# WangWen-Believer/DR-SLAM

Measured on AMD Instinct MI355X. Metric: RGB-D frames/sec (extract+match) at 640x480, higher is better.
Workload: dtype u8; 1 GPU; 640x480 synthetic RGB-D (TUM3 intrinsics), ORB extract 1000/1.2/8/20/7 + SearchByProjection(frame k, frame k-1, th=15) on consecutive frames; BASELINE config 2; batch_per_gpu=512, batches_in_flight_per_gpu=3, distinct_resident_input_batches_per_gpu=3, sequence_frames_per_rank=64

## Files before the change

dr_slam_amd/csrc/orb_kernels.hip:

```cpp
#include "drfe_internal.h"
#include "../../include/drfe_math.h"

#define WAVE 64

__device__ __forceinline__ int reflect101(int p, int n)
{
    if (p < 0) p = -p;
    if (p >= n) p = 2 * (n - 1) - p;
    return p;
}


#define PYR0_ROWS 2
__global__ __launch_bounds__(256) void k_pyr_level0_wide(const DevLevel L, int pyrSlotBytes, const uint8_t* __restrict__ gray,
                                                         size_t frameStride, size_t rowStride, int x16First, int x16Last,
                                                         uint8_t* __restrict__ pyr)
{
    const int slot = blockIdx.z;
    const int y0 = (blockIdx.y * 4 + threadIdx.y) * PYR0_ROWS;
    const int x16 = x16First + (blockIdx.x * 64 + threadIdx.x) * 16;
    const int bh = L.h + 2 * DRFE_EDGE;
    if (y0 >= bh || x16 > x16Last) return;
    const int sx = x16 - DRFE_EDGE;
    const uint8_t* frame = gray + (size_t)slot * frameStride;
    uint4 out[PYR0_ROWS];
#pragma unroll
    for (int r = 0; r < PYR0_ROWS; r++) {
        const int y = min(y0 + r, bh - 1);
        const uint8_t* src = frame + (size_t)reflect101(y - DRFE_EDGE, L.h) * rowStride;
        const uint4 A = *reinterpret_cast<const uint4*>(src + (sx - 13));
        const uint4 B = *reinterpret_cast<const uint4*>(src + (sx + 3));
        out[r] = make_uint4(__builtin_amdgcn_alignbyte(B.x, A.w, 1), __builtin_amdgcn_alignbyte(B.y, B.x, 1),
                            __builtin_amdgcn_alignbyte(B.z, B.y, 1), __builtin_amdgcn_alignbyte(B.w, B.z, 1));
    }
    uint8_t* dst = pyr + (size_t)slot * pyrSlotBytes + L.pyrOff + x16;
#pragma unroll
    for (int r = 0; r < PYR0_ROWS; r++)
        if (y0 + r < bh) *reinterpret_cast<uint4*>(dst + (size_t)(y0 + r) * L.pyrPitch) = out[r];
}

__global__ __launch_bounds__(256) void k_pyr_level0_edge(const DevLevel L, int pyrSlotBytes, const uint8_t* __restrict__ gray,
                                                         size_t frameStride, size_t rowStride, int leftEnd, int rightBegin,
                                                         uint8_t* __restrict__ pyr)
{
    const int slot = blockIdx.y;
    const int nLeft = leftEnd / 4, nPer = nLeft + (L.pyrPitch - rightBegin) / 4;
    const int bw = L.w + 2 * DRFE_EDGE, bh = L.h + 2 * DRFE_EDGE;
    const int item = blockIdx.x * 256 + threadIdx.x;
    if (item >= nPer * bh) return;
    const int y = item / nPer, t = item - y * nPer;
    const int x4 = t < nLeft ? t * 4 : rightBegin + (t - nLeft) * 4;
    const uint8_t* src = gray + (size_t)slot * frameStride + (size_t)reflect101(y - DRFE_EDGE, L.h) * rowStride;
    uint32_t o = 0;
#pragma unroll
    for (int k = 0; k < 4; k++) {
        const int x = x4 + k;
        uint32_t v = 0;
        if (x < bw) v = src[reflect101(x - DRFE_EDGE, L.w)];
        o |= v << (8 * k);
    }
    *reinterpret_cast<uint32_t*>(pyr + (size_t)slot * pyrSlotBytes + L.pyrOff + (size_t)y * L.pyrPitch + x4) = o;
}

__device__ __forceinline__ uint32_t pick_byte(uint32_t d0, uint32_t d1, uint32_t d2, int o)
{
    const uint32_t w = o < 4 ? d0 : (o < 8 ? d1 : d2);
    return (w >> (8 * (o & 3))) & 0xFFu;
}

#define PYR_ROWS 4
__global__ __launch_bounds__(256) void k_pyr_resize(const DevLevel L, const DevLevel P, int pyrSlotBytes,
                                                    const ResizeTap* __restrict__ taps, uint8_t* __restrict__ pyr)
{
    const int slot = blockIdx.z;
    const int y0 = (blockIdx.y * 4 + threadIdx.y) * PYR_ROWS;
    const int x4 = (blockIdx.x * 64 + threadIdx.x) * 4;
    const int bh = L.h + 2 * DRFE_EDGE;
    if (y0 >= bh || x4 >= L.pyrPitch) return;
    uint8_t* base = pyr + (size_t)slot * pyrSlotBytes;
    const uint4 tya = *reinterpret_cast<const uint4*>(taps + L.ytabOff + y0);
    const uint4 tyb = *reinterpret_cast<const uint4*>(taps + L.ytabOff + y0 + 2);
    const uint4 ta = *reinterpret_cast<const uint4*>(taps + L.xtabOff + x4);
    const uint4 tb = *reinterpret_cast<const uint4*>(taps + L.xtabOff + x4 + 2);
    const uint32_t syp[PYR_ROWS] = {tya.x, tya.z, tyb.x, tyb.z}, wyp[PYR_ROWS] = {tya.y, tya.w, tyb.y, tyb.w};
    const uint32_t sp[4] = {ta.x, ta.z, tb.x, tb.z};
    const uint32_t wp[4] = {ta.y, ta.w, tb.y, tb.w};
    int lo = 0xFFFF;
#pragma unroll
    for (int k = 0; k < 4; k++) lo = min(lo, (int)(sp[k] & 0xFFFF));
    const int ws = (lo + DRFE_EDGE) & ~3;
    const uint8_t* srcw = base + P.pyrOff + (size_t)DRFE_EDGE * P.pyrPitch + ws;
    uint32_t a[PYR_ROWS][3], c[PYR_ROWS][3];
#pragma unroll
    for (int r = 0; r < PYR_ROWS; r++) {
        const uint32_t* R0 = reinterpret_cast<const uint32_t*>(srcw + (size_t)(syp[r] & 0xFFFF) * P.pyrPitch);
        const uint32_t* R1 = reinterpret_cast<const uint32_t*>(srcw + (size_t)(syp[r] >> 16) * P.pyrPitch);
        a[r][0] = R0[0]; a[r][1] = R0[1]; a[r][2] = R0[2];
        c[r][0] = R1[0]; c[r][1] = R1[1]; c[r][2] = R1[2];
    }
    int o0[4], o1[4], w0[4], w1[4];
#pragma unroll
    for (int k = 0; k < 4; k++) {
        o0[k] = (int)(sp[k] & 0xFFFF) + DRFE_EDGE - ws; o1[k] = (int)(sp[k] >> 16) + DRFE_EDGE - ws;
        w0[k] = (int)(short)(wp[k] & 0xFFFF); w1[k] = (int)(short)(wp[k] >> 16);
    }
#pragma unroll
    for (int r = 0; r < PYR_ROWS; r++) {
        if (y0 + r >= bh) break;
        const int b0 = (int)(short)(wyp[r] & 0xFFFF), b1 = (int)(short)(wyp[r] >> 16);
        uint32_t out = 0;
#pragma unroll
        for (int k = 0; k < 4; k++) {
            const int h0 = (int)pick_byte(a[r][0], a[r][1], a[r][2], o0[k]) * w0[k] + (int)pick_byte(a[r][0], a[r][1], a[r][2], o1[k]) * w1[k];
            const int h1 = (int)pick_byte(c[r][0], c[r][1], c[r][2], o0[k]) * w0[k] + (int)pick_byte(c[r][0], c[r][1], c[r][2], o1[k]) * w1[k];
            int v = (((b0 * (h0 >> 4)) >> 16) + ((b1 * (h1 >> 4)) >> 16) + 2) >> 2;
            v = min(255, max(0, v));
            out |= (uint32_t)v << (8 * k);
        }
        *reinterpret_cast<uint32_t*>(base + L.pyrOff + (size_t)(y0 + r) * L.pyrPitch + x4) = out;
    }
}

template <int FILL>
__global__ __launch_bounds__(256) void k_pyr_resize_tile(const DevLevel L, const DevLevel P, int pyrSlotBytes,
                                                         const ResizeTap* __restrict__ taps, uint8_t* __restrict__ pyr,
                                                         uint32_t magicBlocks)
{
    extern __shared__ __attribute__((aligned(16))) uint8_t tile[];
    int bx, slot;
    drfe_xcd_swizzle_2d(magicBlocks, bx, slot);
    bx = __builtin_amdgcn_readfirstlane(bx); slot = __builtin_amdgcn_readfirstlane(slot);
    const int tid = threadIdx.x;
    uint8_t* const base = pyr + (size_t)slot * pyrSlotBytes;
    const uint32_t winp = ((const __attribute__((address_space(4))) uint32_t*)taps)[2 * (L.rzWinOff + bx)];
    const struct { uint32_t s0, s1; } win = {winp & 0xFFFFu, winp >> 16};
    const uint32_t nItems = (uint32_t)(L.rzGroups * L.rzCols);
    uint32_t item = (uint32_t)(bx * DRFE_RESIZE_BLOCK + tid);
    const bool active = item < nItems;
    if (!active) item = nItems - 1;
    auto divm = [](uint32_t n, uint32_t d, uint32_t magic) { const uint32_t q = __umulhi(n, magic); return q * d > n ? q - 1 : q; };
    const uint32_t g = divm(item, (uint32_t)L.rzCols, L.rzColsMagic);
    const int y0 = L.rzRow0 + 4 * (int)g, x4 = 4 * (int)(item - g * (uint32_t)L.rzCols);
    const uint8_t* const tb8 = reinterpret_cast<const uint8_t*>(taps);
    const uint32_t tyo = (uint32_t)(L.ytabOff + y0) * 8u, txo = (uint32_t)(L.xtabOff + x4) * 8u;
    const uint2 t0 = *reinterpret_cast<const uint2*>(tb8 + tyo), t1 = *reinterpret_cast<const uint2*>(tb8 + (tyo + 8u));
    const uint2 t2 = *reinterpret_cast<const uint2*>(tb8 + (tyo + 16u)), t3 = *reinterpret_cast<const uint2*>(tb8 + (tyo + 24u));
    const uint4 ta = *reinterpret_cast<const uint4*>(tb8 + txo);
    const uint4 tb = *reinterpret_cast<const uint4*>(tb8 + (txo + 16u));
    {
        const uint8_t* const srcw = base + P.pyrOff + (uint32_t)((int)win.s0 * P.pyrPitch + (int)win.s1);
        const uint32_t nq = (uint32_t)(L.rzRows * L.rzWq), tpitch = (uint32_t)L.rzWq * 16u;
        uint4 v[FILL];
        uint32_t dst[FILL];
#pragma unroll
        for (int k = 0; k < FILL; k++) {
            const uint32_t j = (uint32_t)tid + (uint32_t)(k * DRFE_RESIZE_BLOCK), jc = j < nq ? j : 0u;
            const uint32_t r = divm(jc, (uint32_t)L.rzWq, L.rzWqMagic), q = jc - r * (uint32_t)L.rzWq;
            v[k] = *reinterpret_cast<const uint4*>(srcw + (__umul24(r, (uint32_t)P.pyrPitch) + q * 16u));
            dst[k] = j < nq ? __umul24(r, tpitch) + q * 16u : nq * 16u;
        }
#pragma unroll
        for (int k = 0; k < FILL; k++) *reinterpret_cast<uint4*>(&tile[dst[k]]) = v[k];
    }
    __syncthreads();
    if (!active) return;
    const uint32_t tpitch = (uint32_t)L.rzWq * 16u;
    const uint32_t sp[4] = {ta.x, ta.z, tb.x, tb.z}, wp[4] = {ta.y, ta.w, tb.y, tb.w};
    int o[4];
#pragma unroll
    for (int k = 0; k < 4; k++) o[k] = (int)(sp[k] & 0xFFFFu) + DRFE_EDGE - (int)win.s1;
    const uint32_t p01 = (uint32_t)min(o[0], o[1]) & ~3u, p23 = (uint32_t)min(o[2], o[3]) & ~3u;
    uint32_t sel[4];
#pragma unroll
    for (int k = 0; k < 4; k++) {
        const uint32_t rel = (uint32_t)o[k] - (k < 2 ? p01 : p23);
        sel[k] = rel | ((rel + 1u) << 16) | 0x0C000C00u;
    }
    typedef unsigned short u16x2v __attribute__((ext_vector_type(2)));
    auto hrow = [&](int srow, uint32_t (&H)[4]) {
        const uint32_t* A = reinterpret_cast<const uint32_t*>(&tile[(uint32_t)srow * tpitch + p01]);
        const uint32_t* C = reinterpret_cast<const uint32_t*>(&tile[(uint32_t)srow * tpitch + p23]);
        const uint32_t a0 = A[0], a1 = A[1], c0 = C[0], c1 = C[1];
        const uint32_t pr[4] = {__builtin_amdgcn_perm(a1, a0, sel[0]), __builtin_amdgcn_perm(a1, a0, sel[1]),
                                __builtin_amdgcn_perm(c1, c0, sel[2]), __builtin_amdgcn_perm(c1, c0, sel[3])};
#pragma unroll
        for (int k = 0; k < 4; k++)
            H[k] = __builtin_amdgcn_udot2(__builtin_bit_cast(u16x2v, pr[k]), __builtin_bit_cast(u16x2v, wp[k]), 0u, false) >> 4;
    };
    uint8_t* const dstLevel = base + L.pyrOff;
    const uint2 typ[4] = {t0, t1, t2, t3};
    const int rowEnd = L.rzRow0 + 4 * L.rzGroups;
    int prevB = -1;
    uint32_t Hp[4] = {0, 0, 0, 0};
#pragma unroll
    for (int r = 0; r < 4; r++) {
        const uint32_t sy = typ[r].x, wy2 = typ[r].y;
        const int a = (int)(sy & 0xFFFFu) + DRFE_EDGE - (int)win.s0, b = (int)(sy >> 16) + DRFE_EDGE - (int)win.s0;
        uint32_t Ha[4], Hb[4];
        if (a == prevB) {
#pragma unroll
            for (int k = 0; k < 4; k++) Ha[k] = Hp[k];
        } else hrow(a, Ha);
        if (b == a) {
#pragma unroll
            for (int k = 0; k < 4; k++) Hb[k] = Ha[k];
        } else hrow(b, Hb);
        const uint32_t b0s = wy2 << 16, b1s = wy2 & 0xFFFF0000u;
        uint32_t sm[4];
#pragma unroll
        for (int k = 0; k < 4; k++) sm[k] = __umulhi(Ha[k], b0s) + __umulhi(Hb[k], b1s) + 2u;
        const u16x2v two = {2, 2};
        const uint32_t q01 = __builtin_bit_cast(uint32_t, __builtin_bit_cast(u16x2v, sm[0] | (sm[1] << 16)) >> two);
        const uint32_t q23 = __builtin_bit_cast(uint32_t, __builtin_bit_cast(u16x2v, sm[2] | (sm[3] << 16)) >> two);
        const uint32_t out = __builtin_amdgcn_perm(q23, q01, 0x06040200u);
        const int y = y0 + r, p = y - DRFE_EDGE;
        *reinterpret_cast<uint32_t*>(dstLevel + (uint32_t)(__umul24((uint32_t)y, (uint32_t)L.pyrPitch) + (uint32_t)x4)) = out;
        if (p >= 1 && p <= DRFE_EDGE && DRFE_EDGE - p < L.rzRow0)
            *reinterpret_cast<uint32_t*>(dstLevel + (uint32_t)(__umul24((uint32_t)(DRFE_EDGE - p), (uint32_t)L.pyrPitch) + (uint32_t)x4)) = out;
        const int yb = DRFE_EDGE + 2 * (L.h - 1) - p;
        if (p >= L.h - 1 - DRFE_EDGE && p <= L.h - 2 && yb >= rowEnd)
            *reinterpret_cast<uint32_t*>(dstLevel + (uint32_t)(__umul24((uint32_t)yb, (uint32_t)L.pyrPitch) + (uint32_t)x4)) = out;
        prevB = b;
#pragma unroll
        for (int k = 0; k < 4; k++) Hp[k] = Hb[k];
    }
}


typedef short s16x2 __attribute__((ext_vector_type(2)));
__device__ __forceinline__ s16x2 pk2(uint32_t lo, uint32_t hi) { return __builtin_bit_cast(s16x2, lo | (hi << 16)); }
__device__ __forceinline__ s16x2 pmin(s16x2 a, s16x2 b) { return __builtin_elementwise_min(a, b); }
__device__ __forceinline__ s16x2 pmax(s16x2 a, s16x2 b) { return __builtin_elementwise_max(a, b); }
typedef unsigned short u16x2 __attribute__((ext_vector_type(2)));
__device__ __forceinline__ u16x2 umax2(u16x2 a, u16x2 b) { return __builtin_elementwise_max(a, b); }
__device__ __forceinline__ u16x2 umin2(u16x2 a, u16x2 b) { return __builtin_elementwise_min(a, b); }

typedef _Float16 h16x2 __attribute__((ext_vector_type(2)));
__device__ __forceinline__ h16x2 hpk(uint32_t lo, uint32_t hi) { return __builtin_bit_cast(h16x2, lo | (hi << 16)); }
__device__ __forceinline__ h16x2 hmin(h16x2 a, h16x2 b) { return __builtin_elementwise_minimum(a, b); }
__device__ __forceinline__ h16x2 hmax(h16x2 a, h16x2 b) { return __builtin_elementwise_maximum(a, b); }
__device__ __forceinline__ h16x2 hmin3(h16x2 a, h16x2 b, h16x2 c) { return hmin(hmin(a, b), c); }
__device__ __forceinline__ h16x2 hmax3(h16x2 a, h16x2 b, h16x2 c) { return hmax(hmax(a, b), c); }

__device__ __forceinline__ h16x2 hpair(const uint8_t* c, int i, int P) { return hpk(c[i], c[i + P]); }
__device__ __forceinline__ uint32_t fast_strength2(const uint8_t* c, const int P)
{
    const int C = 3 * P + 3;
    const h16x2 v = hpair(c, C, P);
    h16x2 d[16];
#define RING(k, o) d[k] = hpair(c, C + (o), P)
    RING(0, 3 * P);       RING(1, 3 * P + 1);   RING(2, 2 * P + 2);    RING(3, P + 3);
    RING(4, 3);           RING(5, -P + 3);      RING(6, -2 * P + 2);   RING(7, -3 * P + 1);
    RING(8, -3 * P);      RING(9, -3 * P - 1);  RING(10, -2 * P - 2);  RING(11, -P - 3);
    RING(12, -3);         RING(13, P - 3);      RING(14, 2 * P - 2);   RING(15, 3 * P - 1);
#undef RING
    h16x2 lo2[8], hi2[8], lo4[8], hi4[8], t[8], u[8];
#pragma unroll
    for (int m = 0; m < 8; m++) {
        lo2[m] = hmin(d[2 * m + 1], d[(2 * m + 2) & 15]);
        hi2[m] = hmax(d[2 * m + 1], d[(2 * m + 2) & 15]);
    }
#pragma unroll
    for (int m = 0; m < 8; m++) { lo4[m] = hmin(lo2[m], lo2[(m + 1) & 7]); hi4[m] = hmax(hi2[m], hi2[(m + 1) & 7]); }
#pragma unroll
    for (int m = 0; m < 8; m++) {
        const h16x2 e0 = d[2 * m], e1 = d[(2 * m + 9) & 15];
        t[m] = hmin3(lo4[m], lo4[(m + 2) & 7], hmax(e0, e1));
        u[m] = hmax3(hi4[m], hi4[(m + 2) & 7], hmin(e0, e1));
    }
    const h16x2 a = hmax(hmax3(hmax3(t[0], t[1], t[2]), t[3], t[4]), hmax3(t[5], t[6], t[7]));
    const h16x2 b = hmin(hmin3(hmin3(u[0], u[1], u[2]), u[3], u[4]), hmin3(u[5], u[6], u[7]));
    const h16x2 one = __builtin_bit_cast(h16x2, 0x00010001u), zero = __builtin_bit_cast(h16x2, 0u);
    const h16x2 r = hmax(hmax(a - v, v - b) - one, zero);
    return __builtin_bit_cast(uint32_t, r);
}

#define FAST_TILE_PITCH 68
#define FAST_MAX_EVAL (DRFE_FAST_MAX_WIN - 6)
#define FAST_SC_PITCH 64

#define FAST_TILE_ROW_BYTES FAST_TILE_PITCH
static inline int fast_sc_off(int maxWh) { return ((maxWh + 1) * FAST_TILE_ROW_BYTES + 15) & ~15; }
static inline int fast_lds_bytes(int maxWh) { return fast_sc_off(maxWh) + (maxWh - 6 + 2) * FAST_SC_PITCH; }

__global__ __launch_bounds__(64) void k_fast_cells(const FastCell* __restrict__ cells, int nlevels, int pyrSlotBytes,
                                                   int candSlotElems, int iniTh, int minTh,
                                                   const uint8_t* __restrict__ pyr, uint32_t* __restrict__ cand0,
                                                   uint32_t* __restrict__ cand1, int* __restrict__ candCount,
                                                   int* __restrict__ status, int scOff, uint32_t gxMagic)
{
    int bx, by;
    drfe_xcd_swizzle_2d(gxMagic, bx, by);
    extern __shared__ __attribute__((aligned(16))) unsigned char fastLds[];
    uint32_t* tile = reinterpret_cast<uint32_t*>(fastLds);
    uint8_t* sc = fastLds + scOff;

    const FastCell fc = cells[bx];
    const int slot = by;
    const int lane = threadIdx.x;
    const int ww = fc.ww, wh = fc.wh;
    const int ew = ww - 6, eh = wh - 6;
    const int off = fc.off;
    const uint8_t* src = pyr + (size_t)slot * pyrSlotBytes + fc.srcOff;
    {
        typedef uint32_t u32x4_a4 __attribute__((ext_vector_type(4), aligned(4)));
        const int nch = (ww + off + 15) >> 4;
        const int c = lane & 3;
        if (c < nch)
            for (int r = lane >> 2; r < wh; r += 16) {
                const u32x4_a4 g = *reinterpret_cast<const u32x4_a4*>(src + (size_t)r * fc.pitch + c * 16);
                uint32_t* t = &tile[r * (FAST_TILE_PITCH / 4) + c * 4];
                t[0] = g.x; t[1] = g.y; t[2] = g.z; t[3] = g.w;
            }
    }
    for (int i = lane; i < (eh + 2) * (FAST_SC_PITCH / 16); i += 64) reinterpret_cast<uint4*>(sc)[i] = make_uint4(0, 0, 0, 0);
    __syncthreads();
    const uint8_t* tb = reinterpret_cast<const uint8_t*>(tile) + off;
    {
        const int nrp = (eh + 1) >> 1;
        const int q64 = 64 / ew, r64 = 64 - q64 * ew;
        int rp = lane / ew, x = lane - rp * ew;
        while (rp < nrp) {
            const int yA = 2 * rp;
            const uint32_t s2 = fast_strength2(&tb[__mul24(yA, FAST_TILE_PITCH) + x], FAST_TILE_PITCH);
            sc[(yA + 1) * FAST_SC_PITCH + (x + 4)] = (uint8_t)(s2 & 0xFF);
            if (2 * rp + 1 < eh) sc[(yA + 2) * FAST_SC_PITCH + (x + 4)] = (uint8_t)(s2 >> 16);
            rp += q64; x += r64;
            if (x >= ew) { x -= ew; rp++; }
        }
    }
    __syncthreads();
    const int nq = (ew + 3) >> 2;
    const uint32_t* scw = reinterpret_cast<const uint32_t*>(sc);
    unsigned long long m20 = 0, m7 = 0;
    {
        const int q64 = 64 / nq, r64 = 64 - q64 * nq;
        int y = lane / nq, q = lane - y * nq;
        const u16x2 thMin = {(unsigned short)(minTh - 1), (unsigned short)(minTh - 1)};
        const u16x2 thIni = {(unsigned short)(iniTh - 1), (unsigned short)(iniTh - 1)};
        const u16x2 one = {1, 1};
        for (int k = 0; y < eh; k += 4) {
            const uint32_t* w = scw + y * (FAST_SC_PITCH / 4) + q;
            u16x2 E[3], O[3], LE[3], RO[3];
#pragma unroll
            for (int r = 0; r < 3; r++) {
                const uint32_t a = w[r * 16], b = w[r * 16 + 1], c = w[r * 16 + 2];
                E[r] = __builtin_bit_cast(u16x2, b & 0x00FF00FFu);
                O[r] = __builtin_bit_cast(u16x2, (b >> 8) & 0x00FF00FFu);
                LE[r] = __builtin_bit_cast(u16x2, __builtin_amdgcn_perm(b, a, 0x0C050C03u));
                RO[r] = __builtin_bit_cast(u16x2, __builtin_amdgcn_perm(c, b, 0x0C040C02u));
            }
            const u16x2 H = umax2(umax2(E[0], O[0]), umax2(E[2], O[2]));
            const u16x2 mE = umax2(umax2(umax2(H, LE[0]), umax2(LE[2], LE[1])), O[1]);
            const u16x2 mO = umax2(umax2(umax2(H, RO[0]), umax2(RO[2], RO[1])), E[1]);
// ... 604 lines not shown
#if defined(DRFE_BLUR_NOSWIZZLE)
    const int bx = blockIdx.x, by = blockIdx.y; (void)gxMagic;
#else
    int bx, by;
    drfe_xcd_swizzle_2d(gxMagic, bx, by);
#endif
    __shared__ __attribute__((aligned(16))) uint32_t hb2[(BLUR_ROWS / 2) * DRFE_BLUR_TW];
    static_assert(BLUR_ROWS % 2 == 0 && DRFE_BLUR_TH % 2 == 0, "row pairs");
    const BlurTile t = tiles[bx];
    const int slot = by, tid = threadIdx.x;
    const DevLevel& L = G->lv[t.level];
    const size_t imgOff = (size_t)__builtin_amdgcn_readfirstlane(slot) * (size_t)G->pyrSlotBytes + (size_t)L.pyrOff;
    const uint8_t* img = pyr + imgOff;
    const int x0 = __builtin_amdgcn_readfirstlane(t.tx * DRFE_BLUR_TW), y0 = __builtin_amdgcn_readfirstlane(t.ty * DRFE_BLUR_TH);
    const int cg = tid & (BLUR_COLG - 1), rr = tid / BLUR_COLG;
    const uint32_t col = (uint32_t)(x0 + cg * 4 + 16);
    const uint32_t pitch = (uint32_t)L.pyrPitch;
    const int lastRow = L.h + 2 * DRFE_EDGE - 1;
#define TAP4(a, b, c, d) ((uint32_t)(a) | ((uint32_t)(b) << 8) | ((uint32_t)(c) << 16) | ((uint32_t)(d) << 24))
    auto hsum4 = [&](uint32_t off, uint32_t (&h)[4]) {
        const uint32_t* row = reinterpret_cast<const uint32_t*>(img + off);
        const uint32_t w0 = row[0], w1 = row[1], w2 = row[2];
        h[0] = __builtin_amdgcn_udot4(w0, TAP4(18, 34, 49, 55), __builtin_amdgcn_udot4(w1, TAP4(49, 34, 18, 0), 0u, false), false);
        h[1] = __builtin_amdgcn_udot4(w0, TAP4(0, 18, 34, 49), __builtin_amdgcn_udot4(w1, TAP4(55, 49, 34, 18), 0u, false), false);
        h[2] = __builtin_amdgcn_udot4(w0, TAP4(0, 0, 18, 34), __builtin_amdgcn_udot4(w1, TAP4(49, 55, 49, 34),
                                      __builtin_amdgcn_udot4(w2, TAP4(18, 0, 0, 0), 0u, false), false), false);
        h[3] = __builtin_amdgcn_udot4(w0, TAP4(0, 0, 0, 18), __builtin_amdgcn_udot4(w1, TAP4(34, 49, 55, 49),
                                      __builtin_amdgcn_udot4(w2, TAP4(34, 18, 0, 0), 0u, false), false), false);
    };
#undef TAP4
    auto pack16 = [](uint32_t lo, uint32_t hi) { return __builtin_amdgcn_perm(hi, lo, 0x05040100u); };
    const int pEnd = __builtin_amdgcn_readfirstlane(min(BLUR_ROWS / 2, (min(DRFE_BLUR_TH, L.h - y0) + 7) >> 1));
    for (int p = rr; p < pEnd; p += BLUR_ROWL) {
        uint32_t ha[4], hc[4];
        const uint32_t ra = (uint32_t)min(y0 + 2 * p - 3 + DRFE_EDGE, lastRow), rc = (uint32_t)min(y0 + 2 * p - 2 + DRFE_EDGE, lastRow);
        hsum4(__umul24(ra, pitch) + col, ha);
        hsum4(__umul24(rc, pitch) + col, hc);
        *reinterpret_cast<uint4*>(&hb2[p * DRFE_BLUR_TW + cg * 4]) =
            make_uint4(pack16(ha[0], hc[0]), pack16(ha[1], hc[1]), pack16(ha[2], hc[2]), pack16(ha[3], hc[3]));
    }
    __syncthreads();
    typedef unsigned short u16x2v __attribute__((ext_vector_type(2)));
    const u16x2v t1834 = {18, 34}, t4955 = {49, 55}, t4934 = {49, 34}, t3449 = {34, 49}, t5549 = {55, 49}, t3418 = {34, 18};
    const int blurPitch = L.blurPitch, levelH = L.h;
    if (x0 + cg * 4 >= blurPitch * DRFE_BTILE_W) return;
    uint8_t* base = blur + (size_t)__builtin_amdgcn_readfirstlane(slot) * (size_t)G->blurSlotBytes + (size_t)L.blurOff;
    for (int q = rr; q < DRFE_BLUR_TH / 2; q += BLUR_ROWL) {
        const int y = y0 + 2 * q;
        if (y >= levelH) continue;
        uint4 P[4];
#pragma unroll
        for (int k = 0; k < 4; k++) P[k] = *reinterpret_cast<const uint4*>(&hb2[(q + k) * DRFE_BLUR_TW + cg * 4]);
        uint32_t a[4], c2v[4];
#pragma unroll
        for (int j = 0; j < 4; j++) {
            const uint32_t p0 = (&P[0].x)[j], p1 = (&P[1].x)[j], p2 = (&P[2].x)[j], p3 = (&P[3].x)[j];
            asm("v_mad_u32_u16 %0, %1, 18, %2" : "=v"(a[j]) : "v"(p3), "s"(32768u));
            a[j] = __builtin_amdgcn_udot2(__builtin_bit_cast(u16x2v, p0), t1834, a[j], false);
            a[j] = __builtin_amdgcn_udot2(__builtin_bit_cast(u16x2v, p1), t4955, a[j], false);
            a[j] = __builtin_amdgcn_udot2(__builtin_bit_cast(u16x2v, p2), t4934, a[j], false);
            asm("v_mad_u32_u16 %0, %1, 18, %2 op_sel:[1,0,0,0]" : "=v"(c2v[j]) : "v"(p0), "s"(32768u));
            c2v[j] = __builtin_amdgcn_udot2(__builtin_bit_cast(u16x2v, p1), t3449, c2v[j], false);
            c2v[j] = __builtin_amdgcn_udot2(__builtin_bit_cast(u16x2v, p2), t5549, c2v[j], false);
            c2v[j] = __builtin_amdgcn_udot2(__builtin_bit_cast(u16x2v, p3), t3418, c2v[j], false);
        }
        const uint32_t outA = pack16((uint32_t)__builtin_amdgcn_ashr_pk_u8_i32((int)a[0], (int)a[1], 16),
                                     (uint32_t)__builtin_amdgcn_ashr_pk_u8_i32((int)a[2], (int)a[3], 16));
        const uint32_t outB = pack16((uint32_t)__builtin_amdgcn_ashr_pk_u8_i32((int)c2v[0], (int)c2v[1], 16),
                                     (uint32_t)__builtin_amdgcn_ashr_pk_u8_i32((int)c2v[2], (int)c2v[3], 16));
        *reinterpret_cast<uint32_t*>(base + drfe_blur_offset(x0 + cg * 4, y, blurPitch)) = outA;
        if (y + 1 < levelH) *reinterpret_cast<uint32_t*>(base + drfe_blur_offset(x0 + cg * 4, y + 1, blurPitch)) = outB;
    }
}


#define DESC_DISC_PER_LANE 12
#ifndef DESC_KPW
#define DESC_KPW 4
#endif
#define DESC_REACH 18
#define DESC_RAW_ROWS 31
#define DESC_RAW_DW 9
#define DESC_BLUR_ROWS (2 * DESC_REACH + 1)
#define DESC_BLUR_DW 10
#define DESC_RAW_N (DESC_RAW_ROWS * DESC_RAW_DW)
#define DESC_BLUR_N (DESC_BLUR_ROWS * DESC_BLUR_DW)
#define DESC_RAW_LD 5
#define DESC_BLUR_LD 6
#define DESC_LDS_DW 372
#ifndef DESC_THREADS
#define DESC_THREADS 64
#endif
#define DESC_WAVES (DESC_THREADS / WAVE)
__global__ __launch_bounds__(DESC_THREADS) void k_orient_desc(const DevGeom* __restrict__ G, const uint8_t* __restrict__ pyr,
                                                     const uint8_t* __restrict__ blur,
                                                     const uint32_t* __restrict__ sel,
                                                     const int* __restrict__ selCount,
                                                     const int8_t* __restrict__ pattern,
                                                     const int16_t* __restrict__ disc, int discCount,
                                                     drfe_keypoint* __restrict__ kps, uint8_t* __restrict__ desc,
                                                     int* __restrict__ kpCount, int maxKp, uint32_t gxMagic)
{
    __shared__ uint32_t sPatch[DESC_WAVES][DESC_KPW][DESC_LDS_DW];
    int bx, by;
    drfe_xcd_swizzle_2d(gxMagic, bx, by);
    const int slot = by;
    const int lane = threadIdx.x & (WAVE - 1);
    const int wv = __builtin_amdgcn_readfirstlane((int)(threadIdx.x >> 6));
    const int g0 = (bx * DESC_WAVES + wv) * DESC_KPW;
    const int nl = G->nlevels;
    const int cntL = lane < nl ? selCount[slot * nl + lane] : 0;
    int incl = cntL;
    incl += __builtin_amdgcn_update_dpp(0, incl, 0x111, 0xf, 0xf, true);
    incl += __builtin_amdgcn_update_dpp(0, incl, 0x112, 0xf, 0xf, true);
    incl += __builtin_amdgcn_update_dpp(0, incl, 0x114, 0xf, 0xf, true);
    incl += __builtin_amdgcn_update_dpp(0, incl, 0x118, 0xf, 0xf, true);
    static_assert(DRFE_MAX_LEVELS == 16, "the level prefix assumes one DPP row");
    const int excl = incl - cntL;
    const int total = __builtin_amdgcn_readlane(incl, DRFE_MAX_LEVELS - 1);
    if (g0 == 0 && lane == 0) kpCount[slot] = min(total, maxKp);
    if (g0 >= total || g0 >= maxKp) return;
    int level[DESC_KPW], xi[DESC_KPW], yi[DESC_KPW], resp[DESC_KPW], pitchP[DESC_KPW], pitchB[DESC_KPW];
    int shP[DESC_KPW], shB[DESC_KPW];
    int bx0[DESC_KPW], by0[DESC_KPW];
    bool live[DESC_KPW];
    const uint8_t* cP[DESC_KPW];
    const uint8_t* cB[DESC_KPW];
    uint32_t key[DESC_KPW];
#pragma unroll
    for (int j = 0; j < DESC_KPW; j++) {
        const int g = g0 + j;
        live[j] = g < total && g < maxKp;
        const int lv = live[j] ? __popcll(__ballot(lane < DRFE_MAX_LEVELS && g >= incl)) : 0;
        const int first = __builtin_amdgcn_readlane(excl, lv);
        level[j] = lv;
        key[j] = live[j] ? sel[(size_t)slot * G->kpSlotElems + G->lv[lv].kpOff + (g - first)] : 0u;
    }
#pragma unroll
    for (int j = 0; j < DESC_KPW; j++) {
        const DevLevel& L = G->lv[level[j]];
        xi[j] = (int)(key[j] & 0xFFF) + L.minBX; yi[j] = (int)((key[j] >> 12) & 0xFFF) + L.minBY;
        resp[j] = (int)(key[j] >> 24);
        pitchP[j] = L.pyrPitch; pitchB[j] = L.blurPitch;
        if (!live[j]) { xi[j] = L.minBX + 16; yi[j] = L.minBY + 16; }
        const size_t oP = (size_t)slot * G->pyrSlotBytes + L.pyrOff + (size_t)(yi[j] + DRFE_EDGE - 15) * L.pyrPitch + (xi[j] + DRFE_EDGE - 15);
        shP[j] = (int)(oP & 3); shB[j] = (xi[j] - DESC_REACH) & 3;
        cP[j] = pyr + (oP & ~(size_t)3);
        cB[j] = blur + (size_t)slot * G->blurSlotBytes + L.blurOff;
        bx0[j] = (xi[j] - DESC_REACH) & ~3; by0[j] = yi[j] - DESC_REACH;
    }
    uint32_t rw[DESC_KPW][DESC_RAW_LD], bw[DESC_KPW][DESC_BLUR_LD];
    {
        int rRow[DESC_RAW_LD], rCol[DESC_RAW_LD], bRow[DESC_BLUR_LD], bCol[DESC_BLUR_LD];
#pragma unroll
        for (int k = 0; k < DESC_RAW_LD; k++) {
            const int t = min(lane + k * WAVE, DESC_RAW_N - 1);
            rRow[k] = (int)(__umul24(t, 7282) >> 16); rCol[k] = (t - __mul24(rRow[k], DESC_RAW_DW)) * 4;
        }
#pragma unroll
        for (int k = 0; k < DESC_BLUR_LD; k++) {
            const int t = min(lane + k * WAVE, DESC_BLUR_N - 1);
            bRow[k] = (int)(__umul24(t, 6554) >> 16); bCol[k] = (t - __mul24(bRow[k], DESC_BLUR_DW)) * 4;
        }
#pragma unroll
        for (int j = 0; j < DESC_KPW; j++) {
#pragma unroll
            for (int k = 0; k < DESC_RAW_LD; k++)
                rw[j][k] = *reinterpret_cast<const uint32_t*>(cP[j] + (uint32_t)(__mul24(rRow[k], pitchP[j]) + rCol[k]));
#pragma unroll
            for (int k = 0; k < DESC_BLUR_LD; k++)
                bw[j][k] = *reinterpret_cast<const uint32_t*>(cB[j] + drfe_blur_offset(bx0[j] + bCol[k], by0[j] + bRow[k], pitchB[j]));
        }
    }
    const uint32_t* disc32 = reinterpret_cast<const uint32_t*>(disc);
    uint32_t uv[DESC_DISC_PER_LANE];
#pragma unroll
    for (int k = 0; k < DESC_DISC_PER_LANE; k++) {
        const int t = lane + k * WAVE;
        uv[k] = t < discCount ? disc32[t] : 0u;
    }
    int m10[DESC_KPW], m01[DESC_KPW];
    {
        int I[DESC_KPW][DESC_DISC_PER_LANE];
        int du[DESC_DISC_PER_LANE], dv[DESC_DISC_PER_LANE];
#pragma unroll
        for (int k = 0; k < DESC_DISC_PER_LANE; k++) { du[k] = (int)(short)(uv[k] & 0xFFFF); dv[k] = (int)(short)(uv[k] >> 16); }
#pragma unroll
        for (int j = 0; j < DESC_KPW; j++)
#pragma unroll
            for (int k = 0; k < DESC_RAW_LD; k++) {
                const int t = lane + k * WAVE;
                if (t < DESC_RAW_N) sPatch[wv][j][t] = rw[j][k];
            }
#pragma unroll
        for (int j = 0; j < DESC_KPW; j++) {
            const uint8_t* pb = reinterpret_cast<const uint8_t*>(sPatch[wv][j]) + shP[j];
#pragma unroll
            for (int k = 0; k < DESC_DISC_PER_LANE; k++) I[j][k] = pb[__mul24(dv[k] + 15, DESC_RAW_DW * 4) + (du[k] + 15)];
        }
#pragma unroll
        for (int j = 0; j < DESC_KPW; j++) {
            m10[j] = 0; m01[j] = 0;
#pragma unroll
            for (int k = 0; k < DESC_DISC_PER_LANE; k++) {
                m10[j] += du[k] * I[j][k];
                m01[j] += dv[k] * I[j][k];
            }
        }
    }
#pragma unroll
    for (int j = 0; j < DESC_KPW; j++) { m10[j] = drfe_wave_sum_i32(m10[j]); m01[j] = drfe_wave_sum_i32(m01[j]); }
    uint32_t pat[4];
#pragma unroll
    for (int r = 0; r < 4; r++) pat[r] = reinterpret_cast<const uint32_t*>(pattern)[r * 64 + lane];
    const float factorPI = (float)(3.1415926535897932384626433832795 / 180.f);
    float angle[DESC_KPW], cosA[DESC_KPW], sinA[DESC_KPW];
    {
        int my01 = 0, my10 = 0;
#pragma unroll
        for (int j = 0; j < DESC_KPW; j++)
            if (lane == j) { my01 = m01[j]; my10 = m10[j]; }
        const float ang = drfe_fast_atan2((float)my01, (float)my10);
        float sn, cs;
        drfe_sincos(ang * factorPI, &sn, &cs);
#pragma unroll
        for (int j = 0; j < DESC_KPW; j++) {
            angle[j] = __builtin_bit_cast(float, __builtin_amdgcn_readlane(__builtin_bit_cast(int, ang), j));
            cosA[j] = __builtin_bit_cast(float, __builtin_amdgcn_readlane(__builtin_bit_cast(int, cs), j));
            sinA[j] = __builtin_bit_cast(float, __builtin_amdgcn_readlane(__builtin_bit_cast(int, sn), j));
        }
    }
#pragma unroll
    for (int j = 0; j < DESC_KPW; j++)
#pragma unroll
        for (int k = 0; k < DESC_BLUR_LD; k++) {
            const int t = lane + k * WAVE;
            if (t < DESC_BLUR_N) sPatch[wv][j][t] = bw[j][k];
        }
    typedef float f32x2 __attribute__((ext_vector_type(2)));
    f32x2 PX[4], PY[4];
#pragma unroll
    for (int r = 0; r < 4; r++) {
        const uint32_t q4 = pat[r];
        PX[r] = f32x2{(float)(int8_t)(q4 & 0xFF), (float)(int8_t)((q4 >> 16) & 0xFF)};
        PY[r] = f32x2{(float)(int8_t)((q4 >> 8) & 0xFF), (float)(int8_t)(q4 >> 24)};
    }
    const f32x2 magic = {12582912.0f, 12582912.0f};
    const uint32_t excess = 0x400000u * (DESC_BLUR_DW * 4) + 0x4B400000u;
    int t0[DESC_KPW][4], t1[DESC_KPW][4];
#pragma unroll
    for (int j = 0; j < DESC_KPW; j++) {
        const f32x2 a = {cosA[j], cosA[j]}, b = {sinA[j], sinA[j]};
        const uint8_t* pc = reinterpret_cast<const uint8_t*>(sPatch[wv][j]) + shB[j] + DESC_REACH * (DESC_BLUR_DW * 4) + DESC_REACH;
#pragma unroll
        for (int r = 0; r < 4; r++) {
            const f32x2 ry = (PX[r] * b + PY[r] * a) + magic;
            const f32x2 rx = (PX[r] * a - PY[r] * b) + magic;
            const float ry0 = ry.x, ry1 = ry.y, rx0 = rx.x, rx1 = rx.y;
            const uint32_t i0 = __umul24(__float_as_uint(ry0), DESC_BLUR_DW * 4) + __float_as_uint(rx0) - excess;
            const uint32_t i1 = __umul24(__float_as_uint(ry1), DESC_BLUR_DW * 4) + __float_as_uint(rx1) - excess;
            t0[j][r] = pc[(int)i0];
            t1[j][r] = pc[(int)i1];
        }
    }
#pragma unroll
    for (int j = 0; j < DESC_KPW; j++) {
        unsigned long long w4[4];
#pragma unroll
        for (int r = 0; r < 4; r++) w4[r] = __ballot(t0[j][r] < t1[j][r]);
        if (lane == 0 && live[j]) {
            const int g = g0 + j;
            uint8_t* drow = desc + ((size_t)slot * maxKp + g) * 32;
            reinterpret_cast<ulonglong2*>(drow)[0] = make_ulonglong2(w4[0], w4[1]);
            reinterpret_cast<ulonglong2*>(drow)[1] = make_ulonglong2(w4[2], w4[3]);
            const DevLevel& L = G->lv[level[j]];
            drfe_keypoint kp;
            kp.x = (float)xi[j]; kp.y = (float)yi[j];
            if (level[j] != 0) { kp.x *= L.scale; kp.y *= L.scale; }
            kp.size = L.kpSize;
            kp.angle = angle[j];
            kp.response = (float)resp[j];
            kp.octave = level[j];
            kp.class_id = -1;
            kps[(size_t)slot * maxKp + g] = kp;
        }
    }
}



__global__ void k_clear_counts(int* __restrict__ candCount, int n, int* __restrict__ status)
{
    const int i = blockIdx.x * 256 + threadIdx.x;
    if (i < n) candCount[(size_t)i * DRFE_CC_LINE] = 0;
    if (i == 0) status[0] = 0;
}

hipError_t drfe_launch_orb(drfe_ctx* c, const uint8_t* d_gray, size_t frameStride, size_t rowStride, int nframes,
                           hipStream_t s)
{
    const DevGeom& g = c->geom;
    const int nl = g.nlevels;
    hipError_t e;
    hipLaunchKernelGGL(k_clear_counts, dim3((nframes * DRFE_CC_SLOT / DRFE_CC_LINE + 255) / 256), dim3(256), 0, s, c->d_candCount, nframes * DRFE_CC_SLOT / DRFE_CC_LINE, c->d_status);
    e = hipGetLastError();
    if (e != hipSuccess) return e;

    prof_begin(c, DRFE_STAGE_PYRAMID, s);
    {
        const DevLevel& L = g.lv[0];
        const int bh = L.h + 2 * DRFE_EDGE;
        const bool aligned16 = (((uintptr_t)d_gray | frameStride | rowStride) & 15) == 0;
        int x16First = 32, x16Last = (L.w / 16) * 16, leftEnd = 0, rightBegin = 0;
        if (aligned16 && x16Last >= x16First) {
            const int nWide = (x16Last - x16First) / 16 + 1;
            hipLaunchKernelGGL(k_pyr_level0_wide, dim3((nWide + 63) / 64, (bh + 4 * PYR0_ROWS - 1) / (4 * PYR0_ROWS), nframes),
                               dim3(64, 4), 0, s, L, g.pyrSlotBytes, d_gray, frameStride, rowStride, x16First, x16Last, c->d_pyr);
            leftEnd = x16First; rightBegin = x16Last + 16;
        }
        const int nEdge = leftEnd / 4 + (L.pyrPitch - rightBegin) / 4;
        hipLaunchKernelGGL(k_pyr_level0_edge, dim3((nEdge * bh + 255) / 256, nframes), dim3(256), 0, s, L,
                           g.pyrSlotBytes, d_gray, frameStride, rowStride, leftEnd, rightBegin, c->d_pyr);
    }
    for (int l = 1; l < nl; l++) {
        const DevLevel& L = g.lv[l];
        if (L.resizeLds) {
            typedef void (*ResizeTileFn)(const DevLevel, const DevLevel, int, const ResizeTap*, uint8_t*, uint32_t);
            static const ResizeTileFn fns[DRFE_RESIZE_MAX_FILL] = {k_pyr_resize_tile<1>, k_pyr_resize_tile<2>, k_pyr_resize_tile<3>,
                k_pyr_resize_tile<4>, k_pyr_resize_tile<5>, k_pyr_resize_tile<6>, k_pyr_resize_tile<7>, k_pyr_resize_tile<8>};
            const dim3 grid(L.rzBlocks, nframes);
            hipLaunchKernelGGL(fns[L.rzFill - 1], grid, dim3(DRFE_RESIZE_BLOCK), (size_t)(L.rzRows * L.rzWq * 16 + 16), s, L,
                               g.lv[l - 1], g.pyrSlotBytes, c->d_taps, c->d_pyr, drfe_div_magic(grid.x));
        } else {
            const dim3 grid((L.pyrPitch / 4 + 63) / 64, (L.h + 2 * DRFE_EDGE + 4 * PYR_ROWS - 1) / (4 * PYR_ROWS), nframes);
            hipLaunchKernelGGL(k_pyr_resize, grid, dim3(64, 4), 0, s, L, g.lv[l - 1], g.pyrSlotBytes, c->d_taps, c->d_pyr);
        }
    }
    prof_end(c, DRFE_STAGE_PYRAMID, s);

    prof_begin(c, DRFE_STAGE_FAST, s);
    if (g.fastCols && !c->fastGeneric) {
        const int nSmall = g.fastColsSmall, nBig = g.totalCells - nSmall;
        if (nSmall > 0)
            hipLaunchKernelGGL((k_fast_cells_cols<8>), dim3(nSmall, nframes), dim3(64), (size_t)fastc_lds_bytes(g.fastColsRows, 8 * 64), s,
                               c->d_cells, g.nlevels, g.pyrSlotBytes, g.candSlotElems, g.iniTh, g.minTh, c->d_pyr, c->d_cand0,
                               c->d_cand1, c->d_candCount, c->d_status, drfe_div_magic((uint32_t)nSmall), 0, c->fastScreen, fastc_list_off(g.fastColsRows), fastc_list_cap(g.fastColsRows, 8 * 64));
        if (nBig > 0) {
            prof_end(c, DRFE_STAGE_FAST, s);
            prof_begin(c, DRFE_STAGE_FAST_B, s);
        }
        if (nBig > 0)
            hipLaunchKernelGGL((k_fast_cells_cols<DRFE_FASTC_MAX_RPL>), dim3(nBig, nframes), dim3(64),
                               (size_t)fastc_lds_bytes(g.fastColsRows, DRFE_FASTC_MAX_RPL * 64), s, c->d_cells, g.nlevels, g.pyrSlotBytes, g.candSlotElems,
                               g.iniTh, g.minTh, c->d_pyr, c->d_cand0, c->d_cand1, c->d_candCount, c->d_status,
                               drfe_div_magic((uint32_t)nBig), nSmall, c->fastScreen, fastc_list_off(g.fastColsRows), fastc_list_cap(g.fastColsRows, DRFE_FASTC_MAX_RPL * 64));
        if (nBig > 0) prof_end(c, DRFE_STAGE_FAST_B, s);
        else prof_end(c, DRFE_STAGE_FAST, s);
    } else {
        hipLaunchKernelGGL(k_fast_cells, dim3(g.totalCells, nframes), dim3(64), (size_t)fast_lds_bytes(g.fastMaxWh), s, c->d_cells,
                           g.nlevels, g.pyrSlotBytes, g.candSlotElems, g.iniTh, g.minTh, c->d_pyr,
                           c->d_cand0, c->d_cand1, c->d_candCount, c->d_status, fast_sc_off(g.fastMaxWh),
                           drfe_div_magic((uint32_t)g.totalCells));
        prof_end(c, DRFE_STAGE_FAST, s);
    }

    prof_begin(c, DRFE_STAGE_QUADTREE, s);
    {
        int nBig = 0, capMax = 0;
        for (int l = 0; l < nl; l++) {
            if (g.lv[l].w * g.lv[l].h > 160000 || g.lv[l].kpCap > 256) nBig = l + 1;
            capMax = std::max(capMax, g.lv[l].kpCap);
        }
        if (nl * nframes <= 2 * 256) nBig = nl;
        if (nBig > 0) {
            if (capMax > 256)
                hipLaunchKernelGGL((k_quadtree<512, 16, DRFE_QT_MAX_NODES>), dim3(nBig, nframes), dim3(512), 0, s, c->d_geom, 0,
                                   c->d_cand0, c->d_cand1, c->d_node, c->d_candCount, c->d_sel, c->d_selCount, c->d_status);
            else
                hipLaunchKernelGGL((k_quadtree<512, 16, 256>), dim3(nBig, nframes), dim3(512), 0, s, c->d_geom, 0, c->d_cand0,
                                   c->d_cand1, c->d_node, c->d_candCount, c->d_sel, c->d_selCount, c->d_status);
        }
        if (nBig < nl)
            hipLaunchKernelGGL((k_quadtree<256, 8, 256>), dim3(nl - nBig, nframes), dim3(256), 0, s, c->d_geom, nBig, c->d_cand0,
                               c->d_cand1, c->d_node, c->d_candCount, c->d_sel, c->d_selCount, c->d_status);
    }
    prof_end(c, DRFE_STAGE_QUADTREE, s);

    prof_begin(c, DRFE_STAGE_BLUR, s);
    hipLaunchKernelGGL(k_blur, dim3(g.totalTiles, nframes), dim3(256), 0, s, c->d_geom, c->d_tiles, c->d_pyr,
                       c->d_blur, drfe_div_magic((uint32_t)g.totalTiles));
    prof_end(c, DRFE_STAGE_BLUR, s);

    prof_begin(c, DRFE_STAGE_DESC, s);
    hipLaunchKernelGGL(k_orient_desc, dim3((c->maxKp + DESC_WAVES * DESC_KPW - 1) / (DESC_WAVES * DESC_KPW), nframes), dim3(DESC_THREADS), 0, s, c->d_geom, c->d_pyr,
                       c->d_blur, c->d_sel, c->d_selCount, c->d_pattern, c->d_disc, c->discCount, c->d_kps,
                       c->d_desc, c->d_kpCount, c->maxKp, drfe_div_magic((uint32_t)((c->maxKp + DESC_WAVES * DESC_KPW - 1) / (DESC_WAVES * DESC_KPW))));
    prof_end(c, DRFE_STAGE_DESC, s);
    return hipGetLastError();
}

size_t drfe_quadtree_lds_bytes() { return sizeof(QtShared<512, DRFE_QT_MAX_NODES>); }

void drfe_fastc_list_caps(const DevGeom& g, int caps[2])
{
    caps[0] = fastc_list_cap(g.fastColsRows, 8 * 64);
    caps[1] = fastc_list_cap(g.fastColsRows, DRFE_FASTC_MAX_RPL * 64);
}
```

Before: 280,200 frames/s.

## Fuse level-0 pyramid copy, edge bands and count clearing into one kernel

Replaces the separate count-clear, wide-interior copy and edge-border kernels for pyramid level 0 with a single launch. Each block handles a group of source rows: some threads stream the interior with 16-byte loads and DPP neighbor sharing, the others build the reflected left and right bands with byte permutes. Each loaded source row is written to its mirrored top and bottom border rows as well, so border rows are never re-read. Block size is picked on the host for good lane fill. This cuts two launches and redundant reads, at the cost of more complex indexing and a fallback path for unaligned inputs.

```diff
diff --git a/dr_slam_amd/csrc/orb_kernels.hip b/dr_slam_amd/csrc/orb_kernels.hip
--- a/dr_slam_amd/csrc/orb_kernels.hip
+++ b/dr_slam_amd/csrc/orb_kernels.hip
@@ -12,44 +12,125 @@
 
 
 #define PYR0_ROWS 2
-__global__ __launch_bounds__(256) void k_pyr_level0_wide(const DevLevel L, int pyrSlotBytes, const uint8_t* __restrict__ gray,
-                                                         size_t frameStride, size_t rowStride, int x16First, int x16Last,
-                                                         uint8_t* __restrict__ pyr)
-{
-    const int slot = blockIdx.z;
-    const int y0 = (blockIdx.y * 4 + threadIdx.y) * PYR0_ROWS;
-    const int x16 = x16First + (blockIdx.x * 64 + threadIdx.x) * 16;
-    const int bh = L.h + 2 * DRFE_EDGE;
-    if (y0 >= bh || x16 > x16Last) return;
-    const int sx = x16 - DRFE_EDGE;
-    const uint8_t* frame = gray + (size_t)slot * frameStride;
-    uint4 out[PYR0_ROWS];
-#pragma unroll
-    for (int r = 0; r < PYR0_ROWS; r++) {
-        const int y = min(y0 + r, bh - 1);
-        const uint8_t* src = frame + (size_t)reflect101(y - DRFE_EDGE, L.h) * rowStride;
-        const uint4 A = *reinterpret_cast<const uint4*>(src + (sx - 13));
-        const uint4 B = *reinterpret_cast<const uint4*>(src + (sx + 3));
-        out[r] = make_uint4(__builtin_amdgcn_alignbyte(B.x, A.w, 1), __builtin_amdgcn_alignbyte(B.y, B.x, 1),
-                            __builtin_amdgcn_alignbyte(B.z, B.y, 1), __builtin_amdgcn_alignbyte(B.w, B.z, 1));
-    }
-    uint8_t* dst = pyr + (size_t)slot * pyrSlotBytes + L.pyrOff + x16;
-#pragma unroll
-    for (int r = 0; r < PYR0_ROWS; r++)
-        if (y0 + r < bh) *reinterpret_cast<uint4*>(dst + (size_t)(y0 + r) * L.pyrPitch) = out[r];
+#define PYR0_LEFT 32
+#define PYR0_MAX_BLOCK 512
+__device__ __forceinline__ void pyr0_store(uint8_t* __restrict__ dst, uint32_t pitch, int h, int p, uint32_t x, const uint4 v)
+{
+    *reinterpret_cast<uint4*>(dst + (__umul24((uint32_t)(p + DRFE_EDGE), pitch) + x)) = v;
+    if (p >= 1 && p <= DRFE_EDGE)
+        *reinterpret_cast<uint4*>(dst + (__umul24((uint32_t)(DRFE_EDGE - p), pitch) + x)) = v;
+    if (p >= h - 1 - DRFE_EDGE && p <= h - 2)
+        *reinterpret_cast<uint4*>(dst + (__umul24((uint32_t)(DRFE_EDGE + 2 * (h - 1) - p), pitch) + x)) = v;
+}
+
+__device__ __forceinline__ uint32_t pyr0_pick(const uint32_t (&W)[5], int i)
+{
+    return i == 0 ? W[0] : i == 1 ? W[1] : i == 2 ? W[2] : i == 3 ? W[3] : i == 4 ? W[4] : 0u;
+}
+
+__global__ __launch_bounds__(PYR0_MAX_BLOCK) void k_pyr_level0(const DevLevel L, int pyrSlotBytes, const uint8_t* __restrict__ gray,
+                                                           size_t frameStride, uint32_t rowStride, uint32_t groupsPerBlock, uint32_t streamThreads,
+                                                           uint32_t nWide, uint32_t nWideMagic, uint32_t nBand, uint32_t nBandMagic,
+                                                           uint8_t* __restrict__ pyr, int* __restrict__ candCount,
+                                                           int* __restrict__ status)
+{
+    const uint32_t slot = blockIdx.y, bx = blockIdx.x, tid = threadIdx.x;
+    const uint8_t* const frame = gray + (size_t)slot * frameStride;
+    uint8_t* const dst = pyr + (size_t)slot * pyrSlotBytes + L.pyrOff;
+    const int w = L.w, h = L.h;
+    const uint32_t pitch = (uint32_t)L.pyrPitch;
+    if (bx == 0) {
+        if (tid < DRFE_CC_SLOT / DRFE_CC_LINE) candCount[(size_t)slot * DRFE_CC_SLOT + tid * DRFE_CC_LINE] = 0;
+        if (slot == 0 && tid == 0) status[0] = 0;
+    }
+    const uint32_t g0 = bx * groupsPerBlock;
+    const uint32_t groupsHere = min(groupsPerBlock, (uint32_t)((h + PYR0_ROWS - 1) / PYR0_ROWS) - g0);
+    if (tid < streamThreads) {
+        const uint32_t nItems = groupsHere * nWide;
+        uint32_t item = tid;
+        const bool active = item < nItems;
+        if (!active) item = nItems - 1;
+        const uint32_t ql = drfe_div_by(item, nWide, nWideMagic), c = item - ql * nWide, q = g0 + ql;
+        int p[PYR0_ROWS];
+        uint32_t off[PYR0_ROWS], aw[PYR0_ROWS];
+        uint4 B[PYR0_ROWS];
+#pragma unroll
+        for (int r = 0; r < PYR0_ROWS; r++) {
+            p[r] = min((int)q * PYR0_ROWS + r, h - 1);
+            off[r] = (uint32_t)p[r] * rowStride + 16u * (c + 1u);
+            B[r] = *reinterpret_cast<const uint4*>(frame + off[r]);
+        }
+#pragma unroll
+        for (int r = 0; r < PYR0_ROWS; r++)
+            aw[r] = (uint32_t)__builtin_amdgcn_update_dpp((int)B[r].w, (int)B[r].w, 0x138, 0xf, 0xf, false);
+        if (c == 0 || (tid & (WAVE - 1)) == 0) {
+#pragma unroll
+            for (int r = 0; r < PYR0_ROWS; r++) aw[r] = *reinterpret_cast<const uint32_t*>(frame + (off[r] - 4u));
+        }
+        if (!active) return;
+#pragma unroll
+        for (int r = 0; r < PYR0_ROWS; r++) {
+            if ((int)q * PYR0_ROWS + r >= h) break;
+            const uint4 o = make_uint4(__builtin_amdgcn_alignbyte(B[r].x, aw[r], 1), __builtin_amdgcn_alignbyte(B[r].y, B[r].x, 1),
+                                       __builtin_amdgcn_alignbyte(B[r].z, B[r].y, 1), __builtin_amdgcn_alignbyte(B[r].w, B[r].z, 1));
+            pyr0_store(dst, pitch, h, p[r], PYR0_LEFT + 16u * c, o);
+        }
+    } else {
+        const uint32_t item = tid - streamThreads, row0 = g0 * PYR0_ROWS;
+        if (item >= min(groupsHere * PYR0_ROWS, (uint32_t)h - row0) * nBand) return;
+        const uint32_t prl = drfe_div_by(item, nBand, nBandMagic), t = item - prl * nBand, pr = row0 + prl;
+        const int x16 = 16 * (int)t < PYR0_LEFT ? 16 * (int)t : 16 * (w / 16) + 16 + 16 * (int)t - PYR0_LEFT;
+        const int bw = w + 2 * DRFE_EDGE;
+        int sMin = w - 1;
+        int sx[16];
+#pragma unroll
+        for (int k = 0; k < 16; k++) {
+            const int x = x16 + k;
+            sx[k] = x < bw ? reflect101(x - DRFE_EDGE, w) : -1;
+            if (x < bw) sMin = min(sMin, sx[k]);
+        }
+        const int d0 = sMin >> 2;
+        const uint8_t* const row = frame + pr * rowStride;
+        uint32_t W[5];
+#pragma unroll
+        for (int i = 0; i < 5; i++) {
+            const int a = 4 * (d0 + i);
+            uint32_t v = 0;
+            if (a + 4 <= w) v = *reinterpret_cast<const uint32_t*>(row + a);
+            else {
+#pragma unroll
+                for (int b = 0; b < 4; b++)
+                    if (a + b < w) v |= (uint32_t)row[a + b] << (8 * b);
+            }
+            W[i] = v;
+        }
+        uint32_t o[4];
+#pragma unroll
+        for (int i = 0; i < 4; i++) {
+            int m = 4 * 5;
+#pragma unroll
+            for (int k = 0; k < 4; k++)
+                if (sx[4 * i + k] >= 0) m = min(m, sx[4 * i + k] - 4 * d0);
+            const int pi = m >> 2;
+            uint32_t sel = 0;
+#pragma unroll
+            for (int k = 0; k < 4; k++)
+                sel |= (sx[4 * i + k] >= 0 ? (uint32_t)(sx[4 * i + k] - 4 * d0 - 4 * pi) : 0x0Cu) << (8 * k);
+            o[i] = __builtin_amdgcn_perm(pyr0_pick(W, pi + 1), pyr0_pick(W, pi), sel);
+        }
+        pyr0_store(dst, pitch, h, (int)pr, (uint32_t)x16, make_uint4(o[0], o[1], o[2], o[3]));
+    }
 }
 
 __global__ __launch_bounds__(256) void k_pyr_level0_edge(const DevLevel L, int pyrSlotBytes, const uint8_t* __restrict__ gray,
-                                                         size_t frameStride, size_t rowStride, int leftEnd, int rightBegin,
-                                                         uint8_t* __restrict__ pyr)
+                                                         size_t frameStride, size_t rowStride, uint8_t* __restrict__ pyr)
 {
     const int slot = blockIdx.y;
-    const int nLeft = leftEnd / 4, nPer = nLeft + (L.pyrPitch - rightBegin) / 4;
+    const int nPer = L.pyrPitch / 4;
     const int bw = L.w + 2 * DRFE_EDGE, bh = L.h + 2 * DRFE_EDGE;
     const int item = blockIdx.x * 256 + threadIdx.x;
     if (item >= nPer * bh) return;
-    const int y = item / nPer, t = item - y * nPer;
-    const int x4 = t < nLeft ? t * 4 : rightBegin + (t - nLeft) * 4;
+    const int y = item / nPer, x4 = (item - y * nPer) * 4;
     const uint8_t* src = gray + (size_t)slot * frameStride + (size_t)reflect101(y - DRFE_EDGE, L.h) * rowStride;
     uint32_t o = 0;
 #pragma unroll
@@ -1260,25 +1341,34 @@
     const DevGeom& g = c->geom;
     const int nl = g.nlevels;
     hipError_t e;
-    hipLaunchKernelGGL(k_clear_counts, dim3((nframes * DRFE_CC_SLOT / DRFE_CC_LINE + 255) / 256), dim3(256), 0, s, c->d_candCount, nframes * DRFE_CC_SLOT / DRFE_CC_LINE, c->d_status);
-    e = hipGetLastError();
-    if (e != hipSuccess) return e;
+    const DevLevel& L0 = g.lv[0];
+    const bool aligned16 = (((uintptr_t)d_gray | frameStride | rowStride) & 15) == 0;
+    const bool oneLaunch = aligned16 && L0.w >= 32 && L0.h > DRFE_EDGE && (uint64_t)L0.h * rowStride < (1ull << 32);
+    if (!oneLaunch) {
+        hipLaunchKernelGGL(k_clear_counts, dim3((nframes * DRFE_CC_SLOT / DRFE_CC_LINE + 255) / 256), dim3(256), 0, s, c->d_candCount, nframes * DRFE_CC_SLOT / DRFE_CC_LINE, c->d_status);
+        e = hipGetLastError();
+        if (e != hipSuccess) return e;
+    }
 
     prof_begin(c, DRFE_STAGE_PYRAMID, s);
-    {
-        const DevLevel& L = g.lv[0];
-        const int bh = L.h + 2 * DRFE_EDGE;
-        const bool aligned16 = (((uintptr_t)d_gray | frameStride | rowStride) & 15) == 0;
-        int x16First = 32, x16Last = (L.w / 16) * 16, leftEnd = 0, rightBegin = 0;
-        if (aligned16 && x16Last >= x16First) {
-            const int nWide = (x16Last - x16First) / 16 + 1;
-            hipLaunchKernelGGL(k_pyr_level0_wide, dim3((nWide + 63) / 64, (bh + 4 * PYR0_ROWS - 1) / (4 * PYR0_ROWS), nframes),
-                               dim3(64, 4), 0, s, L, g.pyrSlotBytes, d_gray, frameStride, rowStride, x16First, x16Last, c->d_pyr);
-            leftEnd = x16First; rightBegin = x16Last + 16;
-        }
-        const int nEdge = leftEnd / 4 + (L.pyrPitch - rightBegin) / 4;
-        hipLaunchKernelGGL(k_pyr_level0_edge, dim3((nEdge * bh + 255) / 256, nframes), dim3(256), 0, s, L,
-                           g.pyrSlotBytes, d_gray, frameStride, rowStride, leftEnd, rightBegin, c->d_pyr);
+    if (oneLaunch) {
+        const uint32_t nWide = (uint32_t)(L0.w / 16 - 1), nBand = (uint32_t)(PYR0_LEFT + L0.pyrPitch - (L0.w / 16) * 16 - 16) / 16u;
+        const uint32_t nGroups = (uint32_t)((L0.h + PYR0_ROWS - 1) / PYR0_ROWS);
+        uint32_t G = 1, sThreads = 0, threads = 0;
+        float bestFill = 0.f;
+        for (uint32_t cand = 1; cand <= nGroups && cand <= 64; cand++) {
+            const uint32_t st = (cand * nWide + WAVE - 1) / WAVE * WAVE, bt = (cand * PYR0_ROWS * nBand + WAVE - 1) / WAVE * WAVE;
+            if (cand > 1 && st + bt > PYR0_MAX_BLOCK) break;
+            const float fill = (float)(cand * (nWide + PYR0_ROWS * nBand)) / (float)(st + bt);
+            if (fill > bestFill) { bestFill = fill; G = cand; sThreads = st; threads = st + bt; }
+        }
+        hipLaunchKernelGGL(k_pyr_level0, dim3((nGroups + G - 1) / G, nframes), dim3(threads), 0, s, L0, g.pyrSlotBytes, d_gray,
+                           frameStride, (uint32_t)rowStride, G, sThreads, nWide, drfe_div_magic(nWide), nBand, drfe_div_magic(nBand),
+                           c->d_pyr, c->d_candCount, c->d_status);
+    } else {
+        const int bh = L0.h + 2 * DRFE_EDGE;
+        hipLaunchKernelGGL(k_pyr_level0_edge, dim3((L0.pyrPitch / 4 * bh + 255) / 256, nframes), dim3(256), 0, s, L0,
+                           g.pyrSlotBytes, d_gray, frameStride, rowStride, c->d_pyr);
     }
     for (int l = 1; l < nl; l++) {
         const DevLevel& L = g.lv[l];
```

New measurement: 281,200 frames/s (median of 4 runs). No clear change (+0.3%).
